# Ren-Okubo/diffusion_model

Hardware: AMD Instinct MI355X
Metric: atoms*denoise-steps/sec, 64-atom SiO2 T=1000 (higher is better)
Workload: dtype bf16; 1 GPU; 64-atom SiO2 cells x 256 graphs/GPU, 4-layer EGNN (H=36, W=1024, m=256), T=1000 reverse steps, fully connected (E=1032192/GPU); global_batch=256, parallelism=replicas x1 (no data-path collective)

## Files before the change

diffusion_model_amd/csrc/egnn_forward.hip:

```cpp
#include <stdarg.h>
#include <stdlib.h>

#include "bwd_graph.h"
#include "common.h"
#include "kernels.h"

namespace egnn {

constexpr int kPreNodes = 16;
__device__ __forceinline__ void table_store(float* p, float v) { *p = v; }
__device__ __forceinline__ void table_store(_Float16* p, float v) { *p = (_Float16)fminf(fmaxf(v, -32000.f), 32000.f); }

template <typename TT>
__global__ __launch_bounds__(kThreads) void node_pre_kernel(const float* __restrict__ h, int N, int H,
                                                            const float* __restrict__ w1catT,
                                                            const float* __restrict__ b1cat, int TC,
                                                            TT* __restrict__ table) {
  extern __shared__ __attribute__((aligned(16))) char smem_raw[];
  float* hs = reinterpret_cast<float*>(smem_raw);
  const int n0 = blockIdx.x * kPreNodes;
  for (int i = threadIdx.x; i < kPreNodes * H; i += kThreads) {
    const int n = n0 + i / H;
    hs[i] = n < N ? h[(size_t)n * H + i % H] : 0.f;
  }
// ... 40 lines not shown
    for (int i = 0; i < 16; ++i) acc[j][i] = b;
  }
  constexpr int kMaxKS = 32;
  const int KS = HP2 / 2;
  float bw[4][kMaxKS];
#pragma unroll
  for (int j = 0; j < 4; ++j) {
    const int col = col0 + 32 * j + r;
#pragma unroll
    for (int s = 0; s < kMaxKS; ++s) {
      const int k = 2 * s + hh;
      bw[j][s] = (s < KS && k < H && col < TC) ? w1catT[(size_t)k * TC + col] : 0.f;
    }
  }
#pragma unroll
  for (int s = 0; s < kMaxKS; ++s)
    if (s < KS) {
      const float a = hs[(2 * s + hh) * 33 + r];
#pragma unroll
      for (int j = 0; j < 4; ++j) acc[j] = __builtin_amdgcn_mfma_f32_32x32x2f32(a, bw[j][s], acc[j], 0, 0, 0);
    }
  if constexpr (sizeof(TT) == 2) {
    constexpr int kLd = kPre2Cols + 8;
    __syncthreads();
    TT* stg = reinterpret_cast<TT*>(smem_raw);
#pragma unroll
    for (int j = 0; j < 4; ++j)
#pragma unroll
      for (int i = 0; i < 16; ++i) table_store(stg + acc_row(i, lane) * kLd + wave * 128 + 32 * j + r, acc[j][i]);
    __syncthreads();
    const int cbase = blockIdx.y * kPre2Cols;
    for (int q = threadIdx.x; q < kPre2Nodes * (kPre2Cols / 8); q += kThreads) {
      const int row = q / (kPre2Cols / 8), piece = q % (kPre2Cols / 8), n = n0 + row, col = cbase + 8 * piece;
      if (n < N && col < TC)
        *reinterpret_cast<f32x4*>(table + (size_t)n * TC + col) = *reinterpret_cast<const f32x4*>(stg + row * kLd + 8 * piece);
    }
  } else {
#pragma unroll
    for (int j = 0; j < 4; ++j) {
      const int col = col0 + 32 * j + r;
      if (col < TC) {
#pragma unroll
        for (int i = 0; i < 16; ++i) {
          const int n = n0 + acc_row(i, lane);
          if (n < N) table_store(table + (size_t)n * TC + col, acc[j][i]);
        }
      }
    }
  }
}


constexpr int kPre3Nodes = kHiloNodes;
template <int NBW>
__global__ __launch_bounds__(kThreads) void node_pre_hilo_kernel(const float* __restrict__ h, int N, int H,
                                                                 const bf16x8* __restrict__ w1hl,
                                                                 const float* __restrict__ b1cat, int TC,
                                                                 _Float16* __restrict__ table, int fin_hs,
                                                                 const float* __restrict__ fin_partial,
                                                                 const float* __restrict__ fin_b2h, float* __restrict__ h_write) {
  extern __shared__ __attribute__((aligned(16))) char smem_raw[];
  float* hs = reinterpret_cast<float*>(smem_raw);
  const int n0 = blockIdx.x * kPre3Nodes;
  for (int i = threadIdx.x; i < kPre3Nodes * 48; i += kThreads) {
    const int node = i / 48, k = i % 48, n = n0 + node;
    float v = 0.f;
    if (n < N && k < H) {
      if (fin_hs > 0) {
        float pv[8];
#pragma unroll
        for (int sp = 0; sp < 8; ++sp) pv[sp] = fin_partial[((size_t)(sp < fin_hs ? sp : 0) * N + n) * H + k];
        v = fin_b2h[k];
#pragma unroll
        for (int sp = 0; sp < 8; ++sp) v += sp < fin_hs ? pv[sp] : 0.f;
        if (blockIdx.y == 0) h_write[(size_t)n * H + k] = v;
      } else v = h[(size_t)n * H + k];
    }
    hs[k * 33 + node] = v;
  }
  __syncthreads();
  const int lane = threadIdx.x & 63, wave = threadIdx.x >> 6, r = lane & 31, hh = lane >> 5;
  bf16x8 ahi[3], alo[3];
#pragma unroll
  for (int ks = 0; ks < 3; ++ks)
#pragma unroll
    for (int j = 0; j < 8; ++j) {
      const float v = hs[(16 * ks + 8 * hh + j) * 33 + r];
      const __bf16 hi = (__bf16)v;
      ahi[ks][j] = hi;
      alo[ks][j] = (__bf16)(v - (float)hi);
    }
  const int cb0 = (blockIdx.y * 4 + wave) * NBW;
  constexpr int kLd = 128 + 8;
  constexpr int kPairs = NBW >= 4 ? 2 : NBW / 2;
  _Float16* stg = reinterpret_cast<_Float16*>(smem_raw + 48 * 33 * 4) + (size_t)wave * 32 * kLd;
  for (int half8 = 0; half8 < (NBW + 3) / 4; ++half8) {
#pragma unroll
    for (int pair = 0; pair < kPairs; ++pair) {
      bf16x8 bf[2][3][2];
#pragma unroll
      for (int jb = 0; jb < 2; ++jb) {
        const int cb = cb0 + 4 * half8 + 2 * pair + jb;
        const bool ok = 32 * cb < TC;
#pragma unroll
        for (int ks = 0; ks < 3; ++ks)
#pragma unroll
          for (int q = 0; q < 2; ++q) bf[jb][ks][q] = ok ? w1hl[(((size_t)cb * 3 + ks) * 2 + q) * 64 + lane] : bf16x8{};
      }
#pragma unroll
      for (int jb = 0; jb < 2; ++jb) {
        const int cb = cb0 + 4 * half8 + 2 * pair + jb, col = 32 * cb + r;
        const float b = col < TC ? b1cat[col] : 0.f;
        f32x16 acc;
#pragma unroll
        for (int i = 0; i < 16; ++i) acc[i] = b;
#pragma unroll
        for (int ks = 0; ks < 3; ++ks) {
          acc = __builtin_amdgcn_mfma_f32_32x32x16_bf16(alo[ks], bf[jb][ks][0], acc, 0, 0, 0);
          acc = __builtin_amdgcn_mfma_f32_32x32x16_bf16(ahi[ks], bf[jb][ks][1], acc, 0, 0, 0);
          acc = __builtin_amdgcn_mfma_f32_32x32x16_bf16(ahi[ks], bf[jb][ks][0], acc, 0, 0, 0);
        }
#pragma unroll
        for (int i = 0; i < 16; ++i) table_store(stg + acc_row(i, lane) * kLd + 32 * (2 * pair + jb) + r, acc[i]);
      }
    }
    __builtin_amdgcn_wave_barrier();
    const int cbase = 32 * (cb0 + 4 * half8);
    constexpr int kPieces = 8 * kPairs;
    for (int q = lane; q < 32 * kPieces; q += 64) {
      const int row = q / kPieces, piece = q % kPieces, n = n0 + row, col = cbase + 8 * piece;
      if (n < N && col < TC)
        *reinterpret_cast<f32x4*>(table + (size_t)n * TC + col) = *reinterpret_cast<const f32x4*>(stg + row * kLd + 8 * piece);
    }
    __builtin_amdgcn_wave_barrier();
  }
}

__global__ void node_d2_kernel(const float* __restrict__ x, const int* __restrict__ row_ptr,
                               const int* __restrict__ edge_src, int N, float* __restrict__ node_d2) {
  const int n = blockIdx.x * blockDim.x + threadIdx.x;
  if (n >= N) return;
  const float x0 = x[3 * n], x1 = x[3 * n + 1], x2 = x[3 * n + 2];
  float s = 0.f;
  for (int e = row_ptr[n]; e < row_ptr[n + 1]; ++e) {
    const int j = edge_src[e];
    const float a = x0 - x[3 * j], b = x1 - x[3 * j + 1], c = x2 - x[3 * j + 2];
    s += a * a + b * b + c * c;
  }
  node_d2[n] = s;
}
__global__ __launch_bounds__(kThreads) void graph_sum_kernel(const float* __restrict__ node_d2,
                                                               const int* __restrict__ graph_ptr, int N,
                                                               int per_graph, float* __restrict__ gscale) {
  __shared__ float red[kThreads];
  const int lo = per_graph ? graph_ptr[blockIdx.x] : 0;
  const int hi = per_graph ? graph_ptr[blockIdx.x + 1] : N;
  float s = 0.f;
  for (int n = lo + threadIdx.x; n < hi; n += kThreads) s += node_d2[n];
  red[threadIdx.x] = s;
  __syncthreads();
  for (int w = kThreads / 2; w > 0; w >>= 1) {
    if (threadIdx.x < w) red[threadIdx.x] += red[threadIdx.x + w];
    __syncthreads();
  }
  if (threadIdx.x == 0) gscale[blockIdx.x] = red[0];
}

__global__ __launch_bounds__(kThreads) void graph_sq_sums_kernel(const int* __restrict__ row_ptr, int R,
                                                                   const float* __restrict__ agg_x,
                                                                   const float* __restrict__ part_x,
                                                                   const int* __restrict__ graph_ptr, int N, int per_graph,
                                                                   float* __restrict__ gscale) {
  __shared__ float red[kThreads];
// ... 459 lines not shown
    if ((rc = dev_alloc(&c->part_m, (tiles + 1) * 2 * c->MP))) return rc;
    if ((rc = dev_alloc(&c->part_x, 4 * (tiles + 1) * 2 * 4))) return rc;
    c->cap_tiles = tiles;
  }
  if (!c->stamps) {
    if ((rc = dev_alloc(&c->stamps, (size_t)2 * 8 * 32 * 4))) return rc;
    EGNN_HIP(hipMemset(c->stamps, 0, 2 * 8 * 32 * 4 * 8));
  }
  if ((size_t)c->B > c->cap_graphs) {
    if ((rc = dev_alloc(&c->gscale, (size_t)c->B + 1))) return rc;
    c->cap_graphs = c->B;
  }
  return EGNN_OK;
}

static void prof_begin(egnn_ctx* c, hipStream_t st, int kind) {
  if (!c->prof) return;
  if (c->ev_used + 2 > c->ev.size()) {
    for (int i = 0; i < 2; ++i) {
      hipEvent_t e;
      if (hipEventCreate(&e) != hipSuccess) return;
      c->ev.push_back(e);
    }
    c->ev_kind.push_back(kind);
  } else {
    c->ev_kind[c->ev_used / 2] = kind;
  }
  (void)hipEventRecord(c->ev[c->ev_used], st);
}
static void prof_end(egnn_ctx* c, hipStream_t st) {
  if (!c->prof || c->ev_used + 2 > c->ev.size()) return;
  (void)hipEventRecord(c->ev[c->ev_used + 1], st);
  c->ev_used += 2;
}


int fork_streams(egnn_ctx* c) {
  if (!c->side || c->ev_fork) return EGNN_OK;
  if (hipEventCreateWithFlags(&c->ev_fork, hipEventDisableTiming) != hipSuccess ||
      hipEventCreateWithFlags(&c->ev_join, hipEventDisableTiming) != hipSuccess) return EGNN_EHIP;
  return EGNN_OK;
}

int init_kernel_attributes() {
  static bool done = false;
  if (done) return EGNN_OK;
  EGNN_HIP(hipFuncSetAttribute(reinterpret_cast<const void*>(&edge_kernel<EGNN_PREC_BF16, 2>),
                               hipFuncAttributeMaxDynamicSharedMemorySize, 160 * 1024));
  EGNN_HIP(hipFuncSetAttribute(reinterpret_cast<const void*>(&edge_kernel<EGNN_PREC_F32, 2>),
                               hipFuncAttributeMaxDynamicSharedMemorySize, 160 * 1024));
  EGNN_HIP(hipFuncSetAttribute(reinterpret_cast<const void*>(&node_post_kernel),
                               hipFuncAttributeMaxDynamicSharedMemorySize, 160 * 1024));
  EGNN_HIP(hipFuncSetAttribute(reinterpret_cast<const void*>(&node_pre_hilo_kernel<8>),
                               hipFuncAttributeMaxDynamicSharedMemorySize, 160 * 1024));
  EGNN_HIP(hipFuncSetAttribute(reinterpret_cast<const void*>(&node_pre_hilo_kernel<2>),
                               hipFuncAttributeMaxDynamicSharedMemorySize, 160 * 1024));
  int rc = init_edge_bf16_v3_attributes();
  if (rc) return rc;
  if ((rc = init_edge_bf16_v4_attributes())) return rc;
  if ((rc = init_node_bf16_attributes())) return rc;
  if ((rc = init_edge_dgrad_attributes())) return rc;
  if ((rc = init_edge_dgrad_graph_attributes())) return rc;
  if ((rc = init_edge_x_m16_attributes())) return rc;
  if ((rc = init_edge_bf16x3_attributes())) return rc;
  if ((rc = init_edge_f16c8w_attributes())) return rc;
  done = true;
  return EGNN_OK;
}

template <int PREC, int RB>
static int launch_edge(const EdgeParams& p, int tiles, size_t smem, hipStream_t st) {
  hipLaunchKernelGGL((edge_kernel<PREC, RB>), dim3(tiles), dim3(kThreads), smem, st, p);
  EGNN_HIP(hipGetLastError());
  return EGNN_OK;
}

static ForwardSwitches forward_switches(bool persistent_possible) {
  static const ForwardSwitches fixed = [] {
    ForwardSwitches s;
    if (const char* e = getenv("EGNN_EDGE")) s.edge = atoi(e);
    if (const char* e = getenv("EGNN_SMALL_EDGES")) s.small_edges = atol(e);
    if (const char* e = getenv("EGNN_SMALL64_EDGES")) s.small64_edges = atol(e);
    return s;
  }();
  ForwardSwitches s = fixed;
  if (persistent_possible) {
    const char* e = getenv("EGNN_X_PERSIST");
    s.x_persist = !(e && atoi(e) == 0);
  }
  return s;
}

static void fill_edge_params(egnn_ctx* c, const float* x, EdgeParams& p) {
  memset(&p, 0, sizeof(p));
  p.N = c->N; p.E = c->E;
  p.edge_dst = c->edge_dst; p.edge_src = c->edge_src; p.row_ptr = c->row_ptr;
  p.x = x; p.table = c->table;
  p.TC = c->TC; p.WxP = c->WxP; p.WmP = c->WmP; p.MP = c->MP; p.cbx = c->cbx; p.cbm = c->cbm;
  p.agg_m = c->agg_m; p.agg_x = c->agg_x; p.part_m = c->part_m; p.part_x = c->part_x;
  p.agg_x_stride = (size_t)c->cap_nodes * 4; p.part_x_stride = (c->cap_tiles + 1) * 2 * 4;
  p.stamps = c->stamps;
#ifdef EGNN_DIAG
  static const int dbg = getenv("EGNN_DEBUG") ? atoi(getenv("EGNN_DEBUG")) : 0;
  p.dbg = dbg;
#endif
}
static void set_edge_streams(const LayerPack& lp, EdgePath path, int prec, EdgeParams& p, const float*& w1catT,
                             const float*& b1cat) {
  const bool sc = path != EdgePath::kGeneric;
  w1catT = sc ? lp.w1catT_s : lp.w1catT; b1cat = sc ? lp.b1cat_s : lp.b1cat;
  p.wdx = sc ? lp.wdx_s : lp.wdx; p.wdm = sc ? lp.wdm_s : lp.wdm; p.b2x = sc ? lp.b2x_s : lp.b2x;
  p.w3x = sc ? lp.w3x_s : lp.w3x; p.b2m = sc ? lp.b2m_s : lp.b2m; p.wa = sc ? lp.wa_s : lp.wa;
  p.scal = lp.scal;
  p.w2x = p.w2m = p.w2x16 = p.w2m16 = p.w2x_lo = p.w2m_lo = p.w2x_c8 = p.w2m_c8 = nullptr;
  p.c8_exp = nullptr;
  switch (path) {
    case EdgePath::kGeneric:
      p.w2x = prec == EGNN_PREC_BF16 ? lp.w2x_bf16 : (const void*)lp.w2x_f32;
      p.w2m = prec == EGNN_PREC_BF16 ? lp.w2m_bf16 : (const void*)lp.w2m_f32;
      break;
    case EdgePath::kBf16:
      p.w2x = lp.w2x_bf16s; p.w2m = lp.w2m_bf16s; p.w2x16 = lp.w2x_bf16s16; p.w2m16 = lp.w2m_bf16s16;
      break;
    case EdgePath::kBf16x3:
      p.w2x = lp.w2x_bf16s; p.w2m = lp.w2m_bf16s; p.w2x_lo = lp.w2x_bf16s_lo; p.w2m_lo = lp.w2m_bf16s_lo;
      break;
    case EdgePath::kF16:
      p.w2m = lp.w2m_f16s; p.w2x16 = lp.w2x_f16s16; p.w2m16 = lp.w2m_f16s16;
      break;
    case EdgePath::kF16c8:
      p.w2x = lp.w2x_f16s; p.w2m = lp.w2m_f16s; p.w2x_c8 = lp.w2x_c8w; p.w2m_c8 = lp.w2m_c8w; p.c8_exp = lp.c8_exp;
      break;
  }
}
static int launch_node_pre(egnn_ctx* c, hipStream_t st, int layer, NodePre form, bool half_table, const float* h, const float* w1catT,
                           const float* b1cat) {
  const int N = c->N;
  _Float16* tab16 = reinterpret_cast<_Float16*>(c->table);
  switch (form) {
    case NodePre::kHilo8:
    case NodePre::kHilo2: {
      const int ntile = (N + kPre3Nodes - 1) / kPre3Nodes;
      const size_t sm = (size_t)48 * 33 * 4 + (size_t)4 * 32 * (128 + 8) * 2;
      const bf16x8* w1hl = reinterpret_cast<const bf16x8*>(c->layers[layer].w1hl_bf16);
      const bool fin = c->pend.active && c->pend.h_out == h;
      const int fhs = fin ? c->pend.hs : 0;
      const float* fb = fin ? c->pend.b2h : nullptr;
      float* fw = fin ? c->pend.h_out : nullptr;
      if (fin) c->pend.active = false;
      if (form == NodePre::kHilo8)
        hipLaunchKernelGGL(node_pre_hilo_kernel<8>, dim3(ntile, (c->TC + 1023) / 1024), dim3(kThreads), sm, st, h, N, c->H, w1hl,
                           b1cat, c->TC, tab16, fhs, c->h_partial, fb, fw);
      else
        hipLaunchKernelGGL(node_pre_hilo_kernel<2>, dim3(ntile, (c->TC + 255) / 256), dim3(kThreads), sm, st, h, N, c->H, w1hl,
                           b1cat, c->TC, tab16, fhs, c->h_partial, fb, fw);
      break;
    }
    case NodePre::kMfma: {
      dim3 grid((N + kPre2Nodes - 1) / kPre2Nodes, (c->TC + kPre2Cols - 1) / kPre2Cols);
      const size_t sm = (size_t)((c->H + 1) & ~1) * 33 * sizeof(float);
      const size_t sm16 = (size_t)kPre2Nodes * (kPre2Cols + 8) * 2;
      if (half_table)
        hipLaunchKernelGGL(node_pre_mfma_kernel<_Float16>, grid, dim3(kThreads), sm > sm16 ? sm : sm16, st, h, N, c->H, w1catT, b1cat,
                           c->TC, tab16);
      else
        hipLaunchKernelGGL(node_pre_mfma_kernel<float>, grid, dim3(kThreads), sm, st, h, N, c->H, w1catT, b1cat, c->TC, c->table);
      break;
    }
    case NodePre::kValu: {
      dim3 grid((N + kPreNodes - 1) / kPreNodes, (c->TC + kThreads - 1) / kThreads);
      const size_t sm = (size_t)kPreNodes * c->H * sizeof(float);
      if (half_table) hipLaunchKernelGGL(node_pre_kernel<_Float16>, grid, dim3(kThreads), sm, st, h, N, c->H, w1catT, b1cat, c->TC, tab16);
      else hipLaunchKernelGGL(node_pre_kernel<float>, grid, dim3(kThreads), sm, st, h, N, c->H, w1catT, b1cat, c->TC, c->table);
      break;
    }
  }
  EGNN_HIP(hipGetLastError());
  return EGNN_OK;
}

int backward_recompute_supported(egnn_ctx* c) {
  EdgeParams p;
  const float *w1catT, *b1cat;
  fill_edge_params(c, nullptr, p);
  set_edge_streams(c->layers[0], EdgePath::kBf16, EGNN_PREC_BF16, p, w1catT, b1cat);
  return edge_bf16_v4_supported(p) && edge_bf16_v3_supported(p) && c->Wx == c->WxP && c->Wm == c->WmP && c->M == c->MP;
}
int backward_table(egnn_ctx* c, hipStream_t st, int layer, const float* h) {
  const LayerPack& lp = c->layers[layer];
  return launch_node_pre(c, st, layer, node_pre_form(true, c->N, c->H, c->TC), true, h, lp.w1catT_s, lp.b1cat_s);
}
int backward_recompute(egnn_ctx* c, hipStream_t st, int layer, const float* x, const float* g_sum_x, const float* g_sum_m,
                       int e_first, int n_edges, void* s1x, void* s1m, void* g_a2x, void* g_a2m, float* s_halves,
                       float* g_b2x, float* g_w3, float* g_b3, float* g_b2m, float* g_wa, float* g_ba) {
  EdgeParams p;
  fill_edge_params(c, x, p);
  const float *w1catT, *b1cat;
  set_edge_streams(c->layers[layer], EdgePath::kBf16, EGNN_PREC_BF16, p, w1catT, b1cat);
  p.edge_dst = c->edge_dst + e_first; p.edge_src = c->edge_src + e_first; p.E = n_edges;
  p.g_sum_x = g_sum_x; p.g_sum_m = g_sum_m;
  p.s1_out = s1x; p.g_a2_out = g_a2x; p.s_half_out = s_halves;
  p.g_col_a = g_b2x; p.g_col_b = g_w3; p.g_scalar = g_b3;
  int rc = launch_edge_bf16_v3_x_bwd(p, st);
// ... 389 lines not shown
```

diffusion_model_amd/csrc/node_bf16.hip:

```cpp
#include <stdlib.h>

#include "diag.h"
#include "kernels.h"

namespace egnn {

namespace {

constexpr int kNodes = 32, kThreadsN = 256;
constexpr int kMaxKS1 = 20;
constexpr int kSplitK = 320;
constexpr int kRingD = 10;
__host__ __device__ inline size_t nb_smem_bytes(int K1Q, int OB, bool split = false) {
  const size_t xs = (size_t)(K1Q / 8) * 33 * 16 * (split ? 2 : 1);
  const size_t red = (size_t)4 * OB * 16 * 64 * 4;
  return xs + red;
}

template <int OBT, typename V8 = bf16x8, bool SPLIT = false, bool HS = false>
__global__ __launch_bounds__(kThreadsN, (OBT > 2 ? 1 : 2)) void node_post_bf16_kernel(const PostParams p) {
  typedef typename OpTraits<V8>::elem elem;
  constexpr float kInvW = 1.0f / OpTraits<V8>::wscale;
  if constexpr (OpTraits<V8>::f16) f16_saturate_mode();
  constexpr bool PF = !HS;
  extern __shared__ __attribute__((aligned(16))) char smem[];
  char* Xb = smem;
  const int tid = threadIdx.x, lane = tid & 63, wave = tid >> 6, r = lane & 31, hh = lane >> 5;
  const int n0 = blockIdx.x * kNodes;
  const int K1Q = SPLIT ? kSplitK : p.K1Q;
  const int KS1 = K1Q / 16, OB = p.HP / 32;
  char* Xl = Xb + (size_t)(K1Q / 8) * 33 * 16;
  float* red = reinterpret_cast<float*>(smem + (size_t)(K1Q / 8) * 33 * 16 * (SPLIT ? 2 : 1));

  const V8* w1 = reinterpret_cast<const V8*>(p.w1h_bf16);
  const V8* w2 = reinterpret_cast<const V8*>(p.w2h_bf16p);
  const int KS2 = p.WhP / 16;
  const int hsplit = gridDim.y, hsi = blockIdx.y;
  const int nhb = p.WhP / 32, hb_per_wave = nhb / (4 * hsplit), hb0 = hsi * (nhb / hsplit);
  const V8* w1l = reinterpret_cast<const V8*>(p.w1h_lo);
  const V8* w2l = reinterpret_cast<const V8*>(p.w2h_lo);
  V8 wf[SPLIT ? 1 : kMaxKS1];
  V8 rh[SPLIT ? kRingD : 1], rl[SPLIT ? kRingD : 1];
  if constexpr (SPLIT) {
    const size_t o = ((size_t)(hb0 + wave * hb_per_wave) * (kSplitK / 16)) * 64 + lane;
#pragma unroll
    for (int s = 0; s < kRingD; ++s) { rh[s] = w1[o + (size_t)s * 64]; rl[s] = w1l[o + (size_t)s * 64]; }
  } else {
    const V8* w1b = w1 + ((size_t)(hb0 + wave * hb_per_wave) * KS1) * 64 + lane;
#pragma unroll
    for (int s = 0; s < kMaxKS1; ++s) wf[s] = w1b[(size_t)(s < KS1 ? s : 0) * 64];
  }
  float b1v[16];
  V8 w2f[OBT][2];
  V8 w2g[SPLIT ? OBT : 1][2];
  {
    const int hbf = hb0 + wave * hb_per_wave;
#pragma unroll
    for (int i = 0; i < 16; ++i) b1v[i] = p.b1h[32 * hbf + acc_row(i, lane)];
#pragma unroll
    for (int ob = 0; ob < OBT; ++ob)
#pragma unroll
      for (int s = 0; s < 2; ++s) {
        w2f[ob][s] = w2[((size_t)(ob < OB ? ob : 0) * KS2 + 2 * hbf + s) * 64 + lane];
        if constexpr (SPLIT) w2g[ob][s] = w2l[((size_t)(ob < OB ? ob : 0) * KS2 + 2 * hbf + s) * 64 + lane];
      }
  }

  int* s_t0 = reinterpret_cast<int*>(red);
  int* s_t1 = s_t0 + kNodes;
  if (tid < kNodes) {
    const int n = n0 + tid;
    int t0 = -1, t1 = -1;
    if (n < p.N) {
      const int rp0 = p.row_ptr[n], rp1 = p.row_ptr[n + 1];
      if (rp1 > rp0) { t0 = rp0 / p.R; t1 = (rp1 - 1) / p.R; }
    }
    s_t0[tid] = t0; s_t1[tid] = t1;
  }
  __syncthreads();
  if constexpr (HS) {
    constexpr int kIt = (kNodes * (kMaxKS1 * 16 / 2) + kThreadsN - 1) / kThreadsN;
    constexpr int kBatch = 5;
    static_assert(kIt % kBatch == 0, "batches of equal size");
#pragma unroll
    for (int b0 = 0; b0 < kIt; b0 += kBatch) {
      float va[kBatch][2], vb[kBatch][2];
      bool more = false;
#pragma unroll
      for (int it = 0; it < kBatch; ++it) {
        const int i = min(tid + kThreadsN * (b0 + it), kNodes * (K1Q / 2) - 1);
        const int node = i / (K1Q / 2), kp = i % (K1Q / 2), n = min(n0 + node, p.N - 1);
        const int t0 = s_t0[node], t1 = s_t1[node];
        more |= t1 > t0 + 1;
#pragma unroll
        for (int u = 0; u < 2; ++u) {
          const int k = 2 * kp + u, c = k - p.H;
          const bool is_h = k < p.H, is_m = !is_h && c < p.MP && t0 >= 0;
          const float* a = is_h ? p.h + (size_t)n * p.H + k
                                : (t0 == t1 ? p.agg_m + (size_t)n * p.MP + (is_m ? c : 0) : p.part_m + ((size_t)(is_m ? t0 : 0) * 2 + 1) * p.MP + (is_m ? c : 0));
          const bool two = is_m && t1 > t0;
          const float* b = two ? p.part_m + ((size_t)(t0 + 1) * 2) * p.MP + c : p.h;
          const float x0 = *a, x1 = *b;
          va[it][u] = (is_h || is_m) ? x0 : 0.f;
          vb[it][u] = two ? x1 : 0.f;
        }
      }
#pragma unroll
      for (int it = 0; it < kBatch; ++it) {
        const int i = tid + kThreadsN * (b0 + it);
        if (i < kNodes * (K1Q / 2)) {
          const int node = i / (K1Q / 2), kp = i % (K1Q / 2), n = n0 + node;
          float v[2] = {va[it][0] + vb[it][0], va[it][1] + vb[it][1]};
          if (n >= p.N) v[0] = v[1] = 0.f;
          else if (more) {
            const int t0 = s_t0[node], t1 = s_t1[node];
#pragma unroll
            for (int u = 0; u < 2; ++u) {
              const int c = 2 * kp + u - p.H;
              if (c >= 0 && c < p.MP)
                for (int t = t0 + 2; t <= t1; ++t) v[u] += p.part_m[((size_t)t * 2) * p.MP + c];
            }
          }
          const int k = 2 * kp;
          elem* dst = reinterpret_cast<elem*>(Xb + ((size_t)(k >> 3) * 33 + node) * 16) + (k & 7);
          const elem e0 = (elem)v[0], e1 = (elem)v[1];
          dst[0] = e0;
          dst[1] = e1;
          if constexpr (SPLIT) {
            elem* dl = reinterpret_cast<elem*>(Xl + ((size_t)(k >> 3) * 33 + node) * 16) + (k & 7);
            dl[0] = (elem)(v[0] - (float)e0);
            dl[1] = (elem)(v[1] - (float)e1);
          }
        }
      }
    }
  } else
#pragma unroll 4
  for (int i = tid; i < kNodes * (K1Q / 2); i += kThreadsN) {
    const int node = i / (K1Q / 2), kp = i % (K1Q / 2), n = n0 + node;
    float v[2] = {0.f, 0.f};
    if (n < p.N) {
      const int t0 = s_t0[node], t1 = s_t1[node];
#pragma unroll
      for (int u = 0; u < 2; ++u) {
        const int k = 2 * kp + u;
        if (k < p.H) v[u] = p.h[(size_t)n * p.H + k];
        else if (k - p.H < p.MP && t0 >= 0) {
          const int c = k - p.H;
          if (t0 == t1) v[u] = p.agg_m[(size_t)n * p.MP + c];
          else {
            float a = p.part_m[((size_t)t0 * 2 + 1) * p.MP + c];
            for (int t = t0 + 1; t <= t1; ++t) a += p.part_m[((size_t)t * 2) * p.MP + c];
            v[u] = a;
          }
        }
      }
    }
    const int k = 2 * kp;
    elem* dst = reinterpret_cast<elem*>(Xb + ((size_t)(k >> 3) * 33 + node) * 16) + (k & 7);
    const elem e0 = (elem)v[0], e1 = (elem)v[1];
    dst[0] = e0;
    dst[1] = e1;
    if constexpr (SPLIT) {
      elem* dl = reinterpret_cast<elem*>(Xl + ((size_t)(k >> 3) * 33 + node) * 16) + (k & 7);
      dl[0] = (elem)(v[0] - (float)e0);
      dl[1] = (elem)(v[1] - (float)e1);
    }
  }
  float* gsq = reinterpret_cast<float*>(smem + nb_smem_bytes(K1Q, p.HP / 32, SPLIT));
  if (p.sq_from_agg && blockIdx.y == 0 && !diag::kNpNoNorm) {
    float* red = gsq + kNodes;
    const int node = tid >> 3, n = n0 + node;
    int g = -1, lo = 0, hi = 0;
    if (n < p.N) { g = p.node_graph[n]; lo = p.graph_ptr[g]; hi = p.graph_ptr[g + 1]; }
    if (g >= 0 && hi - lo <= 64) {
      const float sq = graph_sq_sum8(lo, hi, tid & 7, p.row_ptr, p.R, p.agg_x, p.part_x);
      if ((tid & 7) == 0) gsq[node] = sq;
    }
    const int nlast = min(n0 + kNodes, p.N) - 1;
    const int g_first = p.node_graph[n0], g_last = p.node_graph[nlast];
    for (int gg = g_first; gg <= g_last; ++gg) {
      const int glo = p.graph_ptr[gg], ghi = p.graph_ptr[gg + 1];
      if (ghi - glo <= 64) continue;
      float sacc = 0.f;
      for (int m = glo + tid; m < ghi; m += kThreadsN) sacc += node_sq_sum(m, p.row_ptr, p.R, p.agg_x, p.part_x);
      red[tid] = sacc;
      __syncthreads();
      for (int w = kThreadsN / 2; w > 0; w >>= 1) {
        if (tid < w) red[tid] += red[tid + w];
        __syncthreads();
      }
      const float tot = red[0];
      __syncthreads();
      if (g == gg && (tid & 7) == 0) gsq[node] = tot;
    }
    __syncthreads();
  }
  if (blockIdx.y == 0 && tid < kNodes * 3 && !diag::kNpNoNorm) {
    const int node = tid / 3, d = tid % 3, n = n0 + node;
    if (n < p.N) {
      const int t0 = s_t0[node], t1 = s_t1[node];
      const bool has = t0 >= 0, one = t0 == t1;
      const float xin = p.x[3 * n + d];
      float va[4], vb[4];
#pragma unroll
      for (int hs = 0; hs < 4; ++hs) {
        const bool on = has && hs < p.nsplit_x;
        const float* ax = p.agg_x + (size_t)(on ? hs : 0) * p.agg_x_stride;
        const float* px = p.part_x + (size_t)(on ? hs : 0) * p.part_x_stride;
        const float* a = one || !on ? ax + (size_t)n * 4 + d : px + ((size_t)t0 * 2 + 1) * 4 + d;
        const float* b = on && !one ? px + ((size_t)(t0 + 1) * 2) * 4 + d : ax + (size_t)n * 4 + d;
        const float x0 = *a, x1 = *b;
        va[hs] = on ? x0 : 0.f;
        vb[hs] = on && !one ? x1 : 0.f;
      }
      float v = 0.f;
#pragma unroll
      for (int hs = 0; hs < 4; ++hs) {
        float w = va[hs] + vb[hs];
        if (has && hs < p.nsplit_x && t1 > t0 + 1) {
          const float* px = p.part_x + (size_t)hs * p.part_x_stride;
          for (int t = t0 + 2; t <= t1; ++t) w += px[((size_t)t * 2) * 4 + d];
        }
        v += w;
      }
      const float sq = p.sq_from_agg ? gsq[node] : p.gscale[p.per_graph ? p.node_graph[n] : 0];
      const float g = 1.0f / (sqrtf(sq) + 1.0f);
      p.x_out[3 * n + d] = xin + v * g;
    }
  }
  __syncthreads();

  f32x16 oacc[OBT];
#pragma unroll
  for (int ob = 0; ob < OBT; ++ob)
#pragma unroll
    for (int i = 0; i < 16; ++i) oacc[ob][i] = 0.f;

  const char* xfrag = Xb + ((size_t)hh * 33 + r) * 16;
  V8 wn[SPLIT ? 1 : kMaxKS1];
  const char* xfrag_lo = Xl + ((size_t)hh * 33 + r) * 16;
  for (int q = 0; q < (diag::kNpNoMlp ? 0 : hb_per_wave); ++q) {
    const int hb = hb0 + wave * hb_per_wave + q;
    if constexpr (SPLIT) {
    } else if constexpr (PF) {
      const int hbn = q + 1 < hb_per_wave ? hb + 1 : hb;
      const V8* w1b = w1 + ((size_t)hbn * KS1) * 64 + lane;
#pragma unroll
      for (int s = 0; s < kMaxKS1; ++s) wn[s] = w1b[(size_t)(s < KS1 ? s : 0) * 64];
    } else if (q > 0) {
      const V8* w1b = w1 + ((size_t)hb * KS1) * 64 + lane;
#pragma unroll
      for (int s = 0; s < kMaxKS1; ++s) wf[s] = w1b[(size_t)(s < KS1 ? s : 0) * 64];
    }
    f32x16 acc;
#pragma unroll
    for (int i = 0; i < 16; ++i) acc[i] = 0.f;
    if constexpr (SPLIT) {
      const int hbn = q + 1 < hb_per_wave ? hb + 1 : hb;
      const size_t oc = ((size_t)hb * (kSplitK / 16)) * 64 + lane, on = ((size_t)hbn * (kSplitK / 16)) * 64 + lane;
      static_assert((kSplitK / 16) % kRingD == 0, "the ring slot of a k-step must be a compile-time constant");
#pragma unroll 1
      for (int turn = 0; turn < kSplitK / 16 / kRingD; ++turn) {
        const bool last_turn = turn == kSplitK / 16 / kRingD - 1;
        const size_t ofill = last_turn ? on : oc + (size_t)(turn + 1) * kRingD * 64;
#pragma unroll
        for (int u = 0; u < kRingD; ++u) {
// ... 45 lines not shown
          if constexpr (SPLIT) {
            oacc[ob] = mfma32(w2g[ob][s], hf[s], oacc[ob]);
            oacc[ob] = mfma32(w2f[ob][s], hg[s], oacc[ob]);
          }
          oacc[ob] = mfma32(w2f[ob][s], hf[s], oacc[ob]);
        }
      }
    if constexpr (PF && !SPLIT) {
#pragma unroll
      for (int s = 0; s < kMaxKS1; ++s) wf[s] = wn[s];
    }
  }
#pragma unroll
  for (int ob = 0; ob < OBT; ++ob)
    if (ob < OB) {
#pragma unroll
      for (int i = 0; i < 16; ++i) red[((size_t)(wave * OB + ob) * 16 + i) * 64 + lane] = oacc[ob][i];
    }
  __syncthreads();
  for (int e = tid; e < OB * 16 * 64; e += kThreadsN) {
    const int l = e & 63, i = (e >> 6) & 15, ob = e >> 10;
    float v = 0.f;
#pragma unroll
    for (int w = 0; w < 4; ++w) v += red[((size_t)(w * OB + ob) * 16 + i) * 64 + l];
    if constexpr (OpTraits<V8>::f16) v *= kInvW;
    const int o = 32 * ob + acc_row(i, l), n = n0 + (l & 31);
    if (n < p.N && o < p.H) {
      if (hsplit == 1) p.h_out[(size_t)n * p.H + o] = v + p.b2h[o];
      else p.h_partial[((size_t)hsi * p.N + n) * p.H + o] = v;
    }
  }
}

__global__ void node_post_finish_kernel(int N, int H, int hsplit, const float* __restrict__ partial,
                                        const float* __restrict__ b2h, float* __restrict__ h_out) {
  const int i = blockIdx.x * blockDim.x + threadIdx.x;
  if (i >= N * H) return;
  float pv[8];
#pragma unroll
  for (int s = 0; s < 8; ++s) pv[s] = partial[(size_t)(s < hsplit ? s : 0) * N * H + i];
  float v = b2h[i % H];
#pragma unroll
  for (int s = 0; s < 8; ++s) v += s < hsplit ? pv[s] : 0.f;
  h_out[i] = v;
}

}

int init_node_bf16_attributes() {
  const void* fns[] = {reinterpret_cast<const void*>(&node_post_bf16_kernel<2>),
                       reinterpret_cast<const void*>(&node_post_bf16_kernel<kPostMaxOB>),
                       reinterpret_cast<const void*>(&node_post_bf16_kernel<2, f16x8, true>),
                       reinterpret_cast<const void*>(&node_post_bf16_kernel<2, bf16x8, false, true>),
                       reinterpret_cast<const void*>(&node_post_bf16_kernel<2, f16x8, true, true>)};
  for (const void* f : fns) EGNN_HIP(hipFuncSetAttribute(f, hipFuncAttributeMaxDynamicSharedMemorySize, 160 * 1024));
  return EGNN_OK;
}

bool node_post_bf16_supported(const PostParams& q) {
  return q.w1h_bf16 && q.w2h_bf16p && q.WhP % 128 == 0 && q.HP / 32 <= kPostMaxOB && q.K1Q / 16 <= kMaxKS1 &&
         nb_smem_bytes(q.K1Q, q.HP / 32) + (kNodes + kThreadsN) * 4 <= 160 * 1024;
}

bool node_post_split_supported(const PostParams& q) {
  return q.w1h_lo && q.w2h_lo && q.w1h_bf16 && q.w2h_bf16p && q.HP <= 64 && q.H + q.MP > kSplitK / 2 && q.H + q.MP <= kSplitK &&
         q.WhP % 128 == 0 && nb_smem_bytes(kSplitK, q.HP / 32, true) + (kNodes + kThreadsN) * 4 <= 80 * 1024;
}
int node_post_split_k() { return kSplitK; }

int launch_node_post_finish(int N, int H, int hs, const float* partial, const float* b2h, float* h_out, hipStream_t st) {
  hipLaunchKernelGGL(node_post_finish_kernel, dim3((N * H + 255) / 256), dim3(256), 0, st, N, H, hs, partial, b2h, h_out);
  EGNN_HIP(hipGetLastError());
  return EGNN_OK;
}

int launch_node_post_bf16(const PostParams& q, hipStream_t st, bool split, bool defer_finish, int* hs_out) {
  const int tiles = (q.N + kNodes - 1) / kNodes;
  int hs = 1;
  if (q.h_partial && tiles * 8 <= 256 && (q.WhP / 32) % 32 == 0) hs = 8;
  const dim3 grid(tiles, hs);
  const size_t sm = nb_smem_bytes(split ? kSplitK : q.K1Q, q.HP / 32, split) + (kNodes + kThreadsN) * 4;
  const bool hsk = hs > 1 && q.N >= kNodes;
  if (split) {
    if (hsk) hipLaunchKernelGGL((node_post_bf16_kernel<2, f16x8, true, true>), grid, dim3(kThreadsN), sm, st, q);
    else hipLaunchKernelGGL((node_post_bf16_kernel<2, f16x8, true>), grid, dim3(kThreadsN), sm, st, q);
  } else if (hsk && q.HP <= 64) {
    hipLaunchKernelGGL((node_post_bf16_kernel<2, bf16x8, false, true>), grid, dim3(kThreadsN), sm, st, q);
  } else if (q.HP <= 64) hipLaunchKernelGGL(node_post_bf16_kernel<2>, grid, dim3(kThreadsN), sm, st, q);
  else hipLaunchKernelGGL(node_post_bf16_kernel<kPostMaxOB>, grid, dim3(kThreadsN), sm, st, q);
  if (hs_out) *hs_out = hs;
  if (hs > 1 && !defer_finish)
    hipLaunchKernelGGL(node_post_finish_kernel, dim3((q.N * q.H + 255) / 256), dim3(256), 0, st, q.N, q.H, hs, q.h_partial,
                       q.b2h, q.h_out);
  EGNN_HIP(hipGetLastError());
  return EGNN_OK;
}

}
```

Baseline: 1.715 million atoms*denoise-steps/s.

## Widen node-pre tile to 64 nodes and vectorize/hoist node-post gathers

The node-pre hi/lo GEMM gains a WIDE variant in which each workgroup covers 64 nodes, so every loaded weight fragment is reused across two 32-row tiles, and h is loaded with 16-byte vector reads. The node-post kernel gains gather modes that hoist row_ptr, coordinate and graph-norm loads ahead of the main gather, issue them early so their latency overlaps, and use float4 vector gathers when alignment allows. Both paths are on by default and can be turned off with EGNN_NODE_GATHER=0. The cost is higher register pressure and more template variants, which may reduce occupancy.

Result: no change. 1.716 million atoms*denoise-steps/s, median of 4 (+0.0%).

```diff
diff --git a/diffusion_model_amd/csrc/egnn_forward.hip b/diffusion_model_amd/csrc/egnn_forward.hip
--- a/diffusion_model_amd/csrc/egnn_forward.hip
+++ b/diffusion_model_amd/csrc/egnn_forward.hip
@@ -116,7 +116,7 @@
 
 
 constexpr int kPre3Nodes = kHiloNodes;
-template <int NBW>
+template <int NBW, bool WIDE = false>
 __global__ __launch_bounds__(kThreads) void node_pre_hilo_kernel(const float* __restrict__ h, int N, int H,
                                                                  const bf16x8* __restrict__ w1hl,
                                                                  const float* __restrict__ b1cat, int TC,
@@ -124,9 +124,31 @@
                                                                  const float* __restrict__ fin_partial,
                                                                  const float* __restrict__ fin_b2h, float* __restrict__ h_write) {
   extern __shared__ __attribute__((aligned(16))) char smem_raw[];
+  static_assert(!WIDE || NBW == 8, "the 64-node workgroup exists for the 1024-column form");
+  constexpr int NT = WIDE ? 2 : 1, kTileN = kPre3Nodes * NT, kS = kTileN + 1;
   float* hs = reinterpret_cast<float*>(smem_raw);
-  const int n0 = blockIdx.x * kPre3Nodes;
-  for (int i = threadIdx.x; i < kPre3Nodes * 48; i += kThreads) {
+  const int n0 = blockIdx.x * kTileN;
+  const bool vec_h = WIDE && fin_hs == 0 && H % 4 == 0 && (reinterpret_cast<uintptr_t>(h) & 15) == 0;
+  if constexpr (WIDE) if (vec_h) {
+    constexpr int kQ = kTileN * 12 / kThreads;
+    static_assert(kTileN * 12 % kThreads == 0, "quads per thread");
+    f32x4 qv[kQ];
+#pragma unroll
+    for (int it = 0; it < kQ; ++it) {
+      const int q = threadIdx.x + kThreads * it, node = q / 12, k4 = 4 * (q % 12), n = n0 + node;
+      const bool ok = n < N && k4 < H;
+      qv[it] = *reinterpret_cast<const f32x4*>(h + (ok ? (size_t)n * H + k4 : 0));
+    }
+#pragma unroll
+    for (int it = 0; it < kQ; ++it) {
+      const int q = threadIdx.x + kThreads * it, node = q / 12, k4 = 4 * (q % 12), n = n0 + node;
+      const bool ok = n < N && k4 < H;
+#pragma unroll
+      for (int u = 0; u < 4; ++u) hs[(k4 + u) * kS + node] = ok ? qv[it][u] : 0.f;
+    }
+  }
+  if (!vec_h)
+  for (int i = threadIdx.x; i < kTileN * 48; i += kThreads) {
     const int node = i / 48, k = i % 48, n = n0 + node;
     float v = 0.f;
     if (n < N && k < H) {
@@ -140,24 +162,68 @@
         if (blockIdx.y == 0) h_write[(size_t)n * H + k] = v;
       } else v = h[(size_t)n * H + k];
     }
-    hs[k * 33 + node] = v;
+    hs[k * kS + node] = v;
   }
   __syncthreads();
   const int lane = threadIdx.x & 63, wave = threadIdx.x >> 6, r = lane & 31, hh = lane >> 5;
-  bf16x8 ahi[3], alo[3];
+  bf16x8 ahi[NT][3], alo[NT][3];
+#pragma unroll
+  for (int t = 0; t < NT; ++t)
 #pragma unroll
   for (int ks = 0; ks < 3; ++ks)
 #pragma unroll
     for (int j = 0; j < 8; ++j) {
-      const float v = hs[(16 * ks + 8 * hh + j) * 33 + r];
+      const float v = hs[(16 * ks + 8 * hh + j) * kS + 32 * t + r];
       const __bf16 hi = (__bf16)v;
-      ahi[ks][j] = hi;
-      alo[ks][j] = (__bf16)(v - (float)hi);
+      ahi[t][ks][j] = hi;
+      alo[t][ks][j] = (__bf16)(v - (float)hi);
     }
   const int cb0 = (blockIdx.y * 4 + wave) * NBW;
   constexpr int kLd = 128 + 8;
   constexpr int kPairs = NBW >= 4 ? 2 : NBW / 2;
-  _Float16* stg = reinterpret_cast<_Float16*>(smem_raw + 48 * 33 * 4) + (size_t)wave * 32 * kLd;
+  _Float16* stg = reinterpret_cast<_Float16*>(smem_raw + 48 * kS * 4) + (size_t)wave * 32 * kLd;
+  if constexpr (WIDE) {
+    for (int half8 = 0; half8 < NBW / 4; ++half8) {
+      bf16x8 bf[4][3][2];
+      float bias[4];
+#pragma unroll
+      for (int jb = 0; jb < 4; ++jb) {
+        const int cb = cb0 + 4 * half8 + jb, col = 32 * cb + r;
+        const bool ok = 32 * cb < TC;
+#pragma unroll
+        for (int ks = 0; ks < 3; ++ks)
+#pragma unroll
+          for (int q = 0; q < 2; ++q) bf[jb][ks][q] = ok ? w1hl[(((size_t)cb * 3 + ks) * 2 + q) * 64 + lane] : bf16x8{};
+        bias[jb] = col < TC ? b1cat[col] : 0.f;
+      }
+      const int cbase = 32 * (cb0 + 4 * half8);
+#pragma unroll
+      for (int t = 0; t < NT; ++t) {
+#pragma unroll
+        for (int jb = 0; jb < 4; ++jb) {
+          f32x16 acc;
+#pragma unroll
+          for (int i = 0; i < 16; ++i) acc[i] = bias[jb];
+#pragma unroll
+          for (int ks = 0; ks < 3; ++ks) {
+            acc = __builtin_amdgcn_mfma_f32_32x32x16_bf16(alo[t][ks], bf[jb][ks][0], acc, 0, 0, 0);
+            acc = __builtin_amdgcn_mfma_f32_32x32x16_bf16(ahi[t][ks], bf[jb][ks][1], acc, 0, 0, 0);
+            acc = __builtin_amdgcn_mfma_f32_32x32x16_bf16(ahi[t][ks], bf[jb][ks][0], acc, 0, 0, 0);
+          }
+#pragma unroll
+          for (int i = 0; i < 16; ++i) table_store(stg + acc_row(i, lane) * kLd + 32 * jb + r, acc[i]);
+        }
+        __builtin_amdgcn_wave_barrier();
+        for (int q = lane; q < 32 * 16; q += 64) {
+          const int row = q / 16, piece = q % 16, n = n0 + 32 * t + row, col = cbase + 8 * piece;
+          if (n < N && col < TC)
+            *reinterpret_cast<f32x4*>(table + (size_t)n * TC + col) = *reinterpret_cast<const f32x4*>(stg + row * kLd + 8 * piece);
+        }
+        __builtin_amdgcn_wave_barrier();
+      }
+    }
+    return;
+  }
   for (int half8 = 0; half8 < (NBW + 3) / 4; ++half8) {
 #pragma unroll
     for (int pair = 0; pair < kPairs; ++pair) {
@@ -180,9 +246,9 @@
         for (int i = 0; i < 16; ++i) acc[i] = b;
 #pragma unroll
         for (int ks = 0; ks < 3; ++ks) {
-          acc = __builtin_amdgcn_mfma_f32_32x32x16_bf16(alo[ks], bf[jb][ks][0], acc, 0, 0, 0);
-          acc = __builtin_amdgcn_mfma_f32_32x32x16_bf16(ahi[ks], bf[jb][ks][1], acc, 0, 0, 0);
-          acc = __builtin_amdgcn_mfma_f32_32x32x16_bf16(ahi[ks], bf[jb][ks][0], acc, 0, 0, 0);
+          acc = __builtin_amdgcn_mfma_f32_32x32x16_bf16(alo[0][ks], bf[jb][ks][0], acc, 0, 0, 0);
+          acc = __builtin_amdgcn_mfma_f32_32x32x16_bf16(ahi[0][ks], bf[jb][ks][1], acc, 0, 0, 0);
+          acc = __builtin_amdgcn_mfma_f32_32x32x16_bf16(ahi[0][ks], bf[jb][ks][0], acc, 0, 0, 0);
         }
 #pragma unroll
         for (int i = 0; i < 16; ++i) table_store(stg + acc_row(i, lane) * kLd + 32 * (2 * pair + jb) + r, acc[i]);
@@ -748,6 +814,8 @@
   EGNN_HIP(hipFuncSetAttribute(reinterpret_cast<const void*>(&node_post_kernel),
                                hipFuncAttributeMaxDynamicSharedMemorySize, 160 * 1024));
   EGNN_HIP(hipFuncSetAttribute(reinterpret_cast<const void*>(&node_pre_hilo_kernel<8>),
+                               hipFuncAttributeMaxDynamicSharedMemorySize, 160 * 1024));
+  EGNN_HIP(hipFuncSetAttribute(reinterpret_cast<const void*>(&node_pre_hilo_kernel<8, true>),
                                hipFuncAttributeMaxDynamicSharedMemorySize, 160 * 1024));
   EGNN_HIP(hipFuncSetAttribute(reinterpret_cast<const void*>(&node_pre_hilo_kernel<2>),
                                hipFuncAttributeMaxDynamicSharedMemorySize, 160 * 1024));
@@ -844,7 +912,16 @@
       const float* fb = fin ? c->pend.b2h : nullptr;
       float* fw = fin ? c->pend.h_out : nullptr;
       if (fin) c->pend.active = false;
-      if (form == NodePre::kHilo8)
+      bool wide = false;
+      if (form == NodePre::kHilo8) {
+        const char* e = getenv("EGNN_NODE_GATHER");
+        wide = !(e && atoi(e) == 0);
+      }
+      if (wide)
+        hipLaunchKernelGGL((node_pre_hilo_kernel<8, true>), dim3((N + 2 * kPre3Nodes - 1) / (2 * kPre3Nodes), (c->TC + 1023) / 1024), dim3(kThreads),
+                           (size_t)48 * (2 * kPre3Nodes + 1) * 4 + (size_t)4 * 32 * (128 + 8) * 2, st, h, N, c->H, w1hl, b1cat, c->TC, tab16, fhs,
+                           c->h_partial, fb, fw);
+      else if (form == NodePre::kHilo8)
         hipLaunchKernelGGL(node_pre_hilo_kernel<8>, dim3(ntile, (c->TC + 1023) / 1024), dim3(kThreads), sm, st, h, N, c->H, w1hl,
                            b1cat, c->TC, tab16, fhs, c->h_partial, fb, fw);
       else
diff --git a/diffusion_model_amd/csrc/node_bf16.hip b/diffusion_model_amd/csrc/node_bf16.hip
--- a/diffusion_model_amd/csrc/node_bf16.hip
+++ b/diffusion_model_amd/csrc/node_bf16.hip
@@ -1,3 +1,4 @@
+#include <stdint.h>
 #include <stdlib.h>
 
 #include "diag.h"
@@ -17,11 +18,13 @@
   return xs + red;
 }
 
-template <int OBT, typename V8 = bf16x8, bool SPLIT = false, bool HS = false>
+template <int OBT, typename V8 = bf16x8, bool SPLIT = false, bool HS = false, int GM = HS ? 1 : 0>
 __global__ __launch_bounds__(kThreadsN, (OBT > 2 ? 1 : 2)) void node_post_bf16_kernel(const PostParams p) {
   typedef typename OpTraits<V8>::elem elem;
   constexpr float kInvW = 1.0f / OpTraits<V8>::wscale;
   if constexpr (OpTraits<V8>::f16) f16_saturate_mode();
+  static_assert(!HS || GM == 1, "the hidden-split form has the scalar branch-free gather");
+  constexpr bool HOIST = !HS && GM != 0;
   constexpr bool PF = !HS;
   extern __shared__ __attribute__((aligned(16))) char smem[];
   char* Xb = smem;
@@ -39,6 +42,13 @@
   const int nhb = p.WhP / 32, hb_per_wave = nhb / (4 * hsplit), hb0 = hsi * (nhb / hsplit);
   const V8* w1l = reinterpret_cast<const V8*>(p.w1h_lo);
   const V8* w2l = reinterpret_cast<const V8*>(p.w2h_lo);
+  const bool norm_here = p.sq_from_agg && blockIdx.y == 0 && !diag::kNpNoNorm;
+  int pre_rp0 = 0, pre_rp1 = 0, pre_g = 0;
+  if constexpr (HOIST) {
+    const int nn = min(n0 + (tid & (kNodes - 1)), p.N - 1);
+    pre_rp0 = p.row_ptr[nn]; pre_rp1 = p.row_ptr[nn + 1];
+    if (norm_here) pre_g = p.node_graph[min(n0 + (tid >> 3), p.N - 1)];
+  }
   V8 wf[SPLIT ? 1 : kMaxKS1];
   V8 rh[SPLIT ? kRingD : 1], rl[SPLIT ? kRingD : 1];
   if constexpr (SPLIT) {
@@ -72,15 +82,129 @@
     const int n = n0 + tid;
     int t0 = -1, t1 = -1;
     if (n < p.N) {
-      const int rp0 = p.row_ptr[n], rp1 = p.row_ptr[n + 1];
+      const int rp0 = HOIST ? pre_rp0 : p.row_ptr[n], rp1 = HOIST ? pre_rp1 : p.row_ptr[n + 1];
       if (rp1 > rp0) { t0 = rp0 / p.R; t1 = (rp1 - 1) / p.R; }
     }
     s_t0[tid] = t0; s_t1[tid] = t1;
   }
   __syncthreads();
-  if constexpr (HS) {
+  float* gsq = reinterpret_cast<float*>(smem + nb_smem_bytes(K1Q, p.HP / 32, SPLIT));
+  float cxin = 0.f, cva[4] = {0.f, 0.f, 0.f, 0.f}, cvb[4] = {0.f, 0.f, 0.f, 0.f};
+  int nrp0[8], nrp1[8], nkind[8], nlo = 0, nhi = 0;
+  float nsa[8], nsb[8];
+  bool nsmall = false;
+  if constexpr (HOIST) {
+    {
+      const int node = min(tid / 3, kNodes - 1), d = tid % 3, n = min(n0 + node, p.N - 1);
+      const int t0 = s_t0[node], t1 = s_t1[node];
+      const bool has = t0 >= 0, one = t0 == t1;
+      cxin = p.x[3 * n + d];
+#pragma unroll
+      for (int hs = 0; hs < 4; ++hs) {
+        const bool on = has && hs < p.nsplit_x;
+        const float* ax = p.agg_x + (size_t)(on ? hs : 0) * p.agg_x_stride;
+        const float* px = p.part_x + (size_t)(on ? hs : 0) * p.part_x_stride;
+        const float* a = one || !on ? ax + (size_t)n * 4 + d : px + ((size_t)t0 * 2 + 1) * 4 + d;
+        const float* b = on && !one ? px + ((size_t)(t0 + 1) * 2) * 4 + d : ax + (size_t)n * 4 + d;
+        const float x0 = *a, x1 = *b;
+        cva[hs] = on ? x0 : 0.f;
+        cvb[hs] = on && !one ? x1 : 0.f;
+      }
+    }
+    if (norm_here) {
+      nlo = p.graph_ptr[pre_g]; nhi = p.graph_ptr[pre_g + 1];
+      nsmall = n0 + (tid >> 3) < p.N && nhi - nlo <= 64;
+#pragma unroll
+      for (int k = 0; k < 8; ++k) {
+        const int m = nlo + (tid & 7) + 8 * k, mm = nsmall && m < nhi ? m : nlo;
+        nrp0[k] = p.row_ptr[mm]; nrp1[k] = p.row_ptr[mm + 1];
+      }
+    }
+  }
+  auto norm_request = [&]() {
+    if (!norm_here) return;
+#pragma unroll
+    for (int k = 0; k < 8; ++k) {
+      const int m = nlo + (tid & 7) + 8 * k;
+      const bool ok = nsmall && m < nhi, has = ok && nrp1[k] > nrp0[k];
+      const int t0 = nrp0[k] / p.R, t1 = (nrp1[k] - 1) / p.R;
+      const bool one = t0 == t1;
+      const float* own = p.agg_x + (size_t)(ok ? m : nlo) * 4 + 3;
+      const float* a = !has || one ? own : p.part_x + ((size_t)t0 * 2 + 1) * 4 + 3;
+      const float* b = has && !one ? p.part_x + ((size_t)(t0 + 1) * 2) * 4 + 3 : own;
+      nsa[k] = *a; nsb[k] = *b;
+      nkind[k] = !has ? 0 : one ? 1 : t1 == t0 + 1 ? 2 : 3;
+    }
+  };
+  auto norm_finish = [&]() {
+    if (!norm_here) return;
+    float s = 0.f;
+#pragma unroll
+    for (int k = 0; k < 8; ++k) {
+      float v = nkind[k] == 0 ? 0.f : nkind[k] == 1 ? nsa[k] : nsa[k] + nsb[k];
+      if (nkind[k] == 3) {
+        const int t0 = nrp0[k] / p.R, t1 = (nrp1[k] - 1) / p.R;
+        for (int t = t0 + 2; t <= t1; ++t) v += p.part_x[((size_t)t * 2) * 4 + 3];
+      }
+      s += v;
+    }
+    s += __shfl_xor(s, 1);
+    s += __shfl_xor(s, 2);
+    s += __shfl_xor(s, 4);
+    if (nsmall && (tid & 7) == 0) gsq[tid >> 3] = s;
+  };
+  if constexpr (GM == 2) {
+    typedef elem elem4 __attribute__((ext_vector_type(4)));
+    constexpr int kQIt = kNodes * (kMaxKS1 * 16 / 4) / kThreadsN;
+    constexpr int kQBatch = SPLIT ? 2 : 5;
+    static_assert(kQIt % kQBatch == 0, "batches of equal size");
+    const int QN = K1Q / 4;
+#pragma unroll
+    for (int b0 = 0; b0 < kQIt; b0 += kQBatch) {
+    f32x4 va[kQBatch], vb[kQBatch];
+#pragma unroll
+    for (int it = 0; it < kQBatch; ++it) {
+      const int i = min(tid + kThreadsN * (b0 + it), kNodes * QN - 1);
+      const int node = i / QN, k = 4 * (i % QN), c = k - p.H, n = min(n0 + node, p.N - 1);
+      const int t0 = s_t0[node], t1 = s_t1[node];
+      const bool is_h = k < p.H, is_m = !is_h && c < p.MP && t0 >= 0, two = is_m && t1 > t0;
+      const int cm = is_m ? c : 0;
+      const float* a = is_h ? p.h + (size_t)n * p.H + k
+                            : (t0 == t1 ? p.agg_m + (size_t)n * p.MP + cm : p.part_m + ((size_t)(is_m ? t0 : 0) * 2 + 1) * p.MP + cm);
+      const float* b = two ? p.part_m + ((size_t)(t0 + 1) * 2) * p.MP + c : p.h;
+      va[it] = *reinterpret_cast<const f32x4*>(a);
+      vb[it] = *reinterpret_cast<const f32x4*>(b);
+    }
+    if (b0 == 0) norm_request();
+#pragma unroll
+    for (int it = 0; it < kQBatch; ++it) {
+      const int i = tid + kThreadsN * (b0 + it);
+      if (i < kNodes * QN) {
+        const int node = i / QN, k = 4 * (i % QN), c = k - p.H, n = n0 + node;
+        const int t0 = s_t0[node], t1 = s_t1[node];
+        const bool is_h = k < p.H, is_m = !is_h && c < p.MP && t0 >= 0, two = is_m && t1 > t0;
+        f32x4 v = {0.f, 0.f, 0.f, 0.f};
+        if (n < p.N) {
+          if (two) v = va[it] + vb[it];
+          else if (is_h || is_m) v = va[it];
+          if (is_m && t1 > t0 + 1)
+            for (int t = t0 + 2; t <= t1; ++t) v += *reinterpret_cast<const f32x4*>(p.part_m + ((size_t)t * 2) * p.MP + c);
+        }
+        elem4 e, el;
+#pragma unroll
+        for (int u = 0; u < 4; ++u) {
+          e[u] = (elem)v[u];
+          el[u] = (elem)(v[u] - (float)e[u]);
+        }
+        *reinterpret_cast<elem4*>(reinterpret_cast<elem*>(Xb + ((size_t)(k >> 3) * 33 + node) * 16) + (k & 7)) = e;
+        if constexpr (SPLIT) *reinterpret_cast<elem4*>(reinterpret_cast<elem*>(Xl + ((size_t)(k >> 3) * 33 + node) * 16) + (k & 7)) = el;
+      }
+    }
+    }
+    norm_finish();
+  } else if constexpr (GM == 1) {
     constexpr int kIt = (kNodes * (kMaxKS1 * 16 / 2) + kThreadsN - 1) / kThreadsN;
-    constexpr int kBatch = 5;
+    constexpr int kBatch = HOIST && SPLIT ? 4 : 5;
     static_assert(kIt % kBatch == 0, "batches of equal size");
 #pragma unroll
     for (int b0 = 0; b0 < kIt; b0 += kBatch) {
@@ -105,6 +229,7 @@
           vb[it][u] = two ? x1 : 0.f;
         }
       }
+      if constexpr (HOIST) if (b0 == 0) norm_request();
 #pragma unroll
       for (int it = 0; it < kBatch; ++it) {
         const int i = tid + kThreadsN * (b0 + it);
@@ -134,6 +259,7 @@
         }
       }
     }
+    if constexpr (HOIST) norm_finish();
   } else
 #pragma unroll 4
   for (int i = tid; i < kNodes * (K1Q / 2); i += kThreadsN) {
@@ -167,15 +293,19 @@
       dl[1] = (elem)(v[1] - (float)e1);
     }
   }
-  float* gsq = reinterpret_cast<float*>(smem + nb_smem_bytes(K1Q, p.HP / 32, SPLIT));
-  if (p.sq_from_agg && blockIdx.y == 0 && !diag::kNpNoNorm) {
+  if (norm_here) {
     float* red = gsq + kNodes;
     const int node = tid >> 3, n = n0 + node;
-    int g = -1, lo = 0, hi = 0;
-    if (n < p.N) { g = p.node_graph[n]; lo = p.graph_ptr[g]; hi = p.graph_ptr[g + 1]; }
-    if (g >= 0 && hi - lo <= 64) {
-      const float sq = graph_sq_sum8(lo, hi, tid & 7, p.row_ptr, p.R, p.agg_x, p.part_x);
-      if ((tid & 7) == 0) gsq[node] = sq;
+    int g = -1;
+    if constexpr (HOIST) {
+      if (n < p.N) g = pre_g;
+    } else {
+      int lo = 0, hi = 0;
+      if (n < p.N) { g = p.node_graph[n]; lo = p.graph_ptr[g]; hi = p.graph_ptr[g + 1]; }
+      if (g >= 0 && hi - lo <= 64) {
+        const float sq = graph_sq_sum8(lo, hi, tid & 7, p.row_ptr, p.R, p.agg_x, p.part_x);
+        if ((tid & 7) == 0) gsq[node] = sq;
+      }
     }
     const int nlast = min(n0 + kNodes, p.N) - 1;
     const int g_first = p.node_graph[n0], g_last = p.node_graph[nlast];
@@ -201,18 +331,22 @@
     if (n < p.N) {
       const int t0 = s_t0[node], t1 = s_t1[node];
       const bool has = t0 >= 0, one = t0 == t1;
-      const float xin = p.x[3 * n + d];
+      const float xin = HOIST ? cxin : p.x[3 * n + d];
       float va[4], vb[4];
 #pragma unroll
       for (int hs = 0; hs < 4; ++hs) {
-        const bool on = has && hs < p.nsplit_x;
-        const float* ax = p.agg_x + (size_t)(on ? hs : 0) * p.agg_x_stride;
-        const float* px = p.part_x + (size_t)(on ? hs : 0) * p.part_x_stride;
-        const float* a = one || !on ? ax + (size_t)n * 4 + d : px + ((size_t)t0 * 2 + 1) * 4 + d;
-        const float* b = on && !one ? px + ((size_t)(t0 + 1) * 2) * 4 + d : ax + (size_t)n * 4 + d;
-        const float x0 = *a, x1 = *b;
-        va[hs] = on ? x0 : 0.f;
-        vb[hs] = on && !one ? x1 : 0.f;
+        if constexpr (HOIST) {
+          va[hs] = cva[hs]; vb[hs] = cvb[hs];
+        } else {
+          const bool on = has && hs < p.nsplit_x;
+          const float* ax = p.agg_x + (size_t)(on ? hs : 0) * p.agg_x_stride;
+          const float* px = p.part_x + (size_t)(on ? hs : 0) * p.part_x_stride;
+          const float* a = one || !on ? ax + (size_t)n * 4 + d : px + ((size_t)t0 * 2 + 1) * 4 + d;
+          const float* b = on && !one ? px + ((size_t)(t0 + 1) * 2) * 4 + d : ax + (size_t)n * 4 + d;
+          const float x0 = *a, x1 = *b;
+          va[hs] = on ? x0 : 0.f;
+          vb[hs] = on && !one ? x1 : 0.f;
+        }
       }
       float v = 0.f;
 #pragma unroll
@@ -364,7 +498,11 @@
                        reinterpret_cast<const void*>(&node_post_bf16_kernel<kPostMaxOB>),
                        reinterpret_cast<const void*>(&node_post_bf16_kernel<2, f16x8, true>),
                        reinterpret_cast<const void*>(&node_post_bf16_kernel<2, bf16x8, false, true>),
-                       reinterpret_cast<const void*>(&node_post_bf16_kernel<2, f16x8, true, true>)};
+                       reinterpret_cast<const void*>(&node_post_bf16_kernel<2, f16x8, true, true>),
+                       reinterpret_cast<const void*>(&node_post_bf16_kernel<2, bf16x8, false, false, 1>),
+                       reinterpret_cast<const void*>(&node_post_bf16_kernel<2, bf16x8, false, false, 2>),
+                       reinterpret_cast<const void*>(&node_post_bf16_kernel<2, f16x8, true, false, 1>),
+                       reinterpret_cast<const void*>(&node_post_bf16_kernel<2, f16x8, true, false, 2>)};
   for (const void* f : fns) EGNN_HIP(hipFuncSetAttribute(f, hipFuncAttributeMaxDynamicSharedMemorySize, 160 * 1024));
   return EGNN_OK;
 }
@@ -384,6 +522,13 @@
   hipLaunchKernelGGL(node_post_finish_kernel, dim3((N * H + 255) / 256), dim3(256), 0, st, N, H, hs, partial, b2h, h_out);
   EGNN_HIP(hipGetLastError());
   return EGNN_OK;
+}
+
+template <int OBT, typename V8, bool SPLIT>
+static void launch_throughput(int gm, dim3 grid, size_t sm, hipStream_t st, const PostParams& q) {
+  if (gm == 2) hipLaunchKernelGGL((node_post_bf16_kernel<OBT, V8, SPLIT, false, 2>), grid, dim3(kThreadsN), sm, st, q);
+  else if (gm == 1) hipLaunchKernelGGL((node_post_bf16_kernel<OBT, V8, SPLIT, false, 1>), grid, dim3(kThreadsN), sm, st, q);
+  else hipLaunchKernelGGL((node_post_bf16_kernel<OBT, V8, SPLIT, false, 0>), grid, dim3(kThreadsN), sm, st, q);
 }
 
 int launch_node_post_bf16(const PostParams& q, hipStream_t st, bool split, bool defer_finish, int* hs_out) {
@@ -393,12 +538,19 @@
   const dim3 grid(tiles, hs);
   const size_t sm = nb_smem_bytes(split ? kSplitK : q.K1Q, q.HP / 32, split) + (kNodes + kThreadsN) * 4;
   const bool hsk = hs > 1 && q.N >= kNodes;
+  int gm = 0;
+  if (hs == 1) {
+    const char* e = getenv("EGNN_NODE_GATHER");
+    const bool vec = q.H % 4 == 0 && q.MP % 4 == 0 &&
+                     ((reinterpret_cast<uintptr_t>(q.h) | reinterpret_cast<uintptr_t>(q.agg_m) | reinterpret_cast<uintptr_t>(q.part_m)) & 15) == 0;
+    gm = e && atoi(e) == 0 ? 0 : vec ? 2 : 1;
+  }
   if (split) {
     if (hsk) hipLaunchKernelGGL((node_post_bf16_kernel<2, f16x8, true, true>), grid, dim3(kThreadsN), sm, st, q);
-    else hipLaunchKernelGGL((node_post_bf16_kernel<2, f16x8, true>), grid, dim3(kThreadsN), sm, st, q);
+    else launch_throughput<2, f16x8, true>(gm, grid, sm, st, q);
   } else if (hsk && q.HP <= 64) {
     hipLaunchKernelGGL((node_post_bf16_kernel<2, bf16x8, false, true>), grid, dim3(kThreadsN), sm, st, q);
-  } else if (q.HP <= 64) hipLaunchKernelGGL(node_post_bf16_kernel<2>, grid, dim3(kThreadsN), sm, st, q);
+  } else if (q.HP <= 64) launch_throughput<2, bf16x8, false>(gm, grid, sm, st, q);
   else hipLaunchKernelGGL(node_post_bf16_kernel<kPostMaxOB>, grid, dim3(kThreadsN), sm, st, q);
   if (hs_out) *hs_out = hs;
   if (hs > 1 && !defer_finish)
```
